# feinanshan/TDNet

Measured on AMD Instinct MI355X. Metric: frames/sec (td4-psp18, 1024x2048, full-resolution logits), higher is better.
Workload: dtype f32; 1 GPU; td4-psp18, 1024x2048 Cityscapes-shaped synthetic stream, 3-frame feature cache, 1 clip per GPU; parallelism=clip-parallel x1, RCCL weight broadcast only, target_fps_per_gpu=30

## Files before the change

include/tdnet.h:

```cpp
#ifndef TDNET_H
#define TDNET_H

#include <stddef.h>
#include <stdint.h>

#ifdef __cplusplus
extern "C" {
#endif

typedef struct tdnet tdnet_t;

typedef struct tdnet_cfg {
    int32_t model;
    int32_t backbone;
    int32_t nclass;
    int32_t height;
    int32_t width;
    int32_t device;
} tdnet_cfg;

#define TDNET_WINOGRAD_DEFAULT 3
#define TDNET_ATTENTION_DEFAULT 2
#define TDNET_FUSION_LN_STATS 2
#define TDNET_FUSION_LN_IN_HEAD 4
#define TDNET_FUSION_A_DIRECT 32
#define TDNET_FUSION_DMA_LOADERS 8192
#define TDNET_FUSION_DMA_NARROW 32768
#define TDNET_FUSION_STEM_ROWS 65536
#define TDNET_FUSION_CONV_GROUPS 131072
#define TDNET_FUSION_CLS_IN_HEAD 262144
#define TDNET_FUSION_SPLIT_NARROW 524288
#define TDNET_FUSION_LATE_CHAIN 1048576
#define TDNET_OVERLAP_CHAINS 1
#define TDNET_OVERLAP_LOWREG_TRANSFORMS 2
#define TDNET_OVERLAP_CHAINS_ANY_SIZE 4
#define TDNET_OVERLAP_GEMM_DMA 8
#define TDNET_OVERLAP_VW_SHIFT 4
#define TDNET_OVERLAP_VW_MASK 0x30
#define TDNET_FUSION_DEFAULT (TDNET_FUSION_LN_STATS | TDNET_FUSION_LN_IN_HEAD | TDNET_FUSION_A_DIRECT | TDNET_FUSION_DMA_LOADERS | TDNET_FUSION_DMA_NARROW | \
                              TDNET_FUSION_STEM_ROWS | TDNET_FUSION_CONV_GROUPS | TDNET_FUSION_CLS_IN_HEAD | TDNET_FUSION_SPLIT_NARROW | TDNET_FUSION_LATE_CHAIN)
#define TDNET_FUSION_MASK TDNET_FUSION_DEFAULT
#define TDNET_OVERLAP_DEFAULT (TDNET_OVERLAP_CHAINS | TDNET_OVERLAP_GEMM_DMA | (2 << TDNET_OVERLAP_VW_SHIFT))
#define TDNET_OVERLAP_MASK (TDNET_OVERLAP_CHAINS | TDNET_OVERLAP_LOWREG_TRANSFORMS | TDNET_OVERLAP_CHAINS_ANY_SIZE | TDNET_OVERLAP_GEMM_DMA | TDNET_OVERLAP_VW_MASK)
typedef struct tdnet_opts {
    int32_t winograd;
    int32_t precision;
    int32_t pipeline;
    int32_t gemm_persistent;
    int32_t reserved0;
    int32_t attention;
    int32_t fusion;
    int32_t overlap;
    int32_t reserved[8];
} tdnet_opts;
void tdnet_opts_default(tdnet_opts* o);

typedef struct tdnet_arch {
    int32_t dilated;
    int32_t multi_grid;
    int32_t reserved[6];
} tdnet_arch;
void tdnet_arch_default(tdnet_arch* a);

int  tdnet_create(const tdnet_cfg* cfg, tdnet_t** out);
int  tdnet_create_opts(const tdnet_cfg* cfg, const tdnet_opts* opts , tdnet_t** out);
int  tdnet_create_arch(const tdnet_cfg* cfg, const tdnet_arch* arch , const tdnet_opts* opts ,
                       tdnet_t** out);
int  tdnet_get_opts(const tdnet_t* h, tdnet_opts* out);
int  tdnet_get_arch(const tdnet_t* h, tdnet_arch* out);
int  tdnet_feature_dims(const tdnet_t* h, int* height, int* width);
void tdnet_destroy(tdnet_t* h);

int  tdnet_set_weight(tdnet_t* h, const char* name, const float* host, size_t count);
int  tdnet_finalize_weights(tdnet_t* h);
int  tdnet_create_shared(const tdnet_t* weights_of, const tdnet_opts* opts , tdnet_t** out);
int  tdnet_warmup(tdnet_t* h, void* stream);
int  tdnet_memory_bytes(const tdnet_t* h, size_t* weights_bytes, size_t* handle_bytes);

int  tdnet_forward(tdnet_t* h, const float* img_nchw_dev, int pos_id, float* logits_nchw_dev, void* stream);
int  tdnet_argmax(tdnet_t* h, const float* logits_nchw_dev, int32_t* labels_dev, void* stream);
int  tdnet_forward_labels(tdnet_t* h, const float* img_nchw_dev, int pos_id, int32_t* labels_dev, void* stream);
int  tdnet_set_input_u8(tdnet_t* h, int src_height, int src_width, const double* mean , const double* std );
int  tdnet_forward_u8(tdnet_t* h, const uint8_t* img_hwc_dev, int pos_id, float* logits_nchw_dev, void* stream);
int  tdnet_forward_u8_labels(tdnet_t* h, const uint8_t* img_hwc_dev, int pos_id, uint8_t* labels_dev , void* stream);
int  tdnet_argmax_u8(tdnet_t* h, const float* logits_nchw_dev, uint8_t* labels_dev, void* stream);
int  tdnet_set_output_rgb(tdnet_t* h, int out_height, int out_width, const uint8_t* palette_rgb , int n_colours );
int  tdnet_forward_rgb(tdnet_t* h, const float* img_nchw_dev, int pos_id, uint8_t* rgb_dev, void* stream);
int  tdnet_forward_u8_rgb(tdnet_t* h, const uint8_t* img_hwc_dev, int pos_id, uint8_t* rgb_dev, void* stream);
int  tdnet_labels_rgb(tdnet_t* h, const uint8_t* labels_u8_dev, uint8_t* rgb_dev, void* stream);
int  tdnet_set_score(tdnet_t* h, const uint8_t* gt_map );
int  tdnet_forward_score(tdnet_t* h, const float* img_nchw_dev, int pos_id, const uint8_t* gt_u8_dev, uint8_t* labels_u8_dev , void* stream);
int  tdnet_forward_u8_score(tdnet_t* h, const uint8_t* img_hwc_dev, int pos_id, const uint8_t* gt_u8_dev, uint8_t* labels_u8_dev , void* stream);
int  tdnet_labels_score(tdnet_t* h, const uint8_t* labels_u8_dev, const uint8_t* gt_u8_dev, void* stream);
// ... 34 lines not shown
```

tdnet_amd/_capi.py:

```python
import ctypes
import os

_HERE = os.path.dirname(os.path.abspath(__file__))
DEFAULT_LIB = os.path.join(_HERE, "lib", "libtdnet_hip.so")
TEST_LIB = os.path.join(_HERE, "lib", "libtdnet_hip_test.so")

c_float_p = ctypes.POINTER(ctypes.c_float)
c_void_p = ctypes.c_void_p


class TdnetCfg(ctypes.Structure):
    _fields_ = [("model", ctypes.c_int32), ("backbone", ctypes.c_int32), ("nclass", ctypes.c_int32),
                ("height", ctypes.c_int32), ("width", ctypes.c_int32), ("device", ctypes.c_int32)]


class TdnetOpts(ctypes.Structure):
    _fields_ = [("winograd", ctypes.c_int32), ("precision", ctypes.c_int32), ("pipeline", ctypes.c_int32),
                ("gemm_persistent", ctypes.c_int32), ("reserved0", ctypes.c_int32), ("attention", ctypes.c_int32),
                ("fusion", ctypes.c_int32), ("overlap", ctypes.c_int32), ("reserved", ctypes.c_int32 * 8)]

    def as_dict(self):
        return {k: getattr(self, k) for k, _ in self._fields_ if not k.startswith("reserved")}


# ... 43 lines not shown
    "tdnet_forward_u8_rgb": (ctypes.c_int, [c_void_p, c_void_p, ctypes.c_int, c_void_p, c_void_p]),
    "tdnet_labels_rgb": (ctypes.c_int, [c_void_p, c_void_p, c_void_p, c_void_p]),
    "tdnet_propagate_rgb": (ctypes.c_int, [c_void_p, c_void_p, c_void_p]),
    "tdnet_set_score": (ctypes.c_int, [c_void_p, c_void_p]),
    "tdnet_forward_score": (ctypes.c_int, [c_void_p, c_void_p, ctypes.c_int, c_void_p, c_void_p, c_void_p]),
    "tdnet_forward_u8_score": (ctypes.c_int, [c_void_p, c_void_p, ctypes.c_int, c_void_p, c_void_p, c_void_p]),
    "tdnet_propagate_score": (ctypes.c_int, [c_void_p, c_void_p, c_void_p, c_void_p]),
    "tdnet_labels_score": (ctypes.c_int, [c_void_p, c_void_p, c_void_p, c_void_p]),
    "tdnet_score_reset": (ctypes.c_int, [c_void_p, c_void_p]),
    "tdnet_score_export": (ctypes.c_int, [c_void_p, c_void_p, c_void_p]),
    "tdnet_score_read": (ctypes.c_long, [c_void_p, c_void_p, ctypes.c_size_t, c_void_p]),
    "tdnet_reset": (ctypes.c_int, [c_void_p]),
    "tdnet_fifo_len": (ctypes.c_int, [c_void_p]),
    "tdnet_encode": (ctypes.c_int, [c_void_p, c_void_p, ctypes.c_int, c_void_p]),
    "tdnet_propagate": (ctypes.c_int, [c_void_p, c_void_p, c_void_p]),
    "tdnet_propagate_labels": (ctypes.c_int, [c_void_p, c_void_p, c_void_p]),
    "tdnet_cache_dims": (ctypes.c_int, [c_void_p, ctypes.POINTER(ctypes.c_int), ctypes.POINTER(ctypes.c_int), ctypes.POINTER(ctypes.c_int)]),
    "tdnet_cache_export": (ctypes.c_int, [c_void_p, c_void_p, c_void_p, c_void_p, c_void_p]),
    "tdnet_cache_push": (ctypes.c_int, [c_void_p, c_void_p, c_void_p, c_void_p, c_void_p]),
    "tdnet_get_stage": (ctypes.c_long, [c_void_p, ctypes.c_char_p, c_void_p, ctypes.c_size_t]),
    "tdnet_flops_per_frame": (ctypes.c_double, [c_void_p]),
    "tdnet_set_profiling": (ctypes.c_int, [c_void_p, ctypes.c_int]),
    "tdnet_last_ms": (ctypes.c_double, [c_void_p, ctypes.c_int]),
    "tdnet_last_flops": (ctypes.c_double, [c_void_p, ctypes.c_int]),
    "tdnet_last_launches": (ctypes.c_double, [c_void_p, ctypes.c_int]),
    "tdnet_last_error": (ctypes.c_char_p, []),
    "tdnet_version": (ctypes.c_char_p, []),
}


TEST_SYMBOLS = {
    "tdnet_bench_mfma_peak": (ctypes.c_double, [ctypes.c_int, ctypes.c_int, c_void_p]),
    "tdnet_bench_conv": (ctypes.c_double, [ctypes.c_int] * 9 + [c_opts_p, c_void_p]),
    "tdnet_op_conv2d": (ctypes.c_int, [c_void_p, ctypes.c_int, ctypes.c_int, ctypes.c_int, c_void_p, c_void_p, ctypes.c_int,
                                       ctypes.c_int, ctypes.c_int, ctypes.c_int, c_void_p, ctypes.c_int, c_opts_p, ctypes.c_int,
                                       c_void_p, c_void_p]),
    "tdnet_op_conv2d_f16io": (ctypes.c_int, [c_void_p, ctypes.c_int, ctypes.c_int, ctypes.c_int, c_void_p, c_void_p, ctypes.c_int,
                                             ctypes.c_int, ctypes.c_int, ctypes.c_int, c_void_p, ctypes.c_int, ctypes.c_int,
                                             c_void_p, c_void_p]),
    "tdnet_op_stem": (ctypes.c_int, [c_void_p, ctypes.c_int, ctypes.c_int, c_void_p, c_void_p, c_opts_p, c_void_p, c_void_p]),
    "tdnet_op_attention": (ctypes.c_int, [c_void_p, c_void_p, c_void_p, c_void_p, c_void_p, ctypes.c_int, ctypes.c_int,
                                          ctypes.c_int, ctypes.c_int, c_void_p, c_void_p, c_void_p, c_void_p, c_void_p]),
    "tdnet_op_layernorm_hw": (ctypes.c_int, [c_void_p, ctypes.c_int, ctypes.c_int, c_void_p, c_void_p, c_void_p, c_void_p]),
    "tdnet_op_ppm": (ctypes.c_int, [c_void_p, ctypes.c_int, ctypes.c_int, c_void_p, c_void_p, ctypes.c_int, ctypes.c_int,
                                    c_void_p, c_void_p]),
    "tdnet_op_upsample": (ctypes.c_int, [c_void_p, ctypes.c_int, ctypes.c_int, ctypes.c_int, ctypes.c_int, ctypes.c_int,
                                         c_void_p, c_void_p]),
    "tdnet_op_stem_image": (ctypes.c_long, [c_void_p, c_void_p, ctypes.c_int, ctypes.c_int, ctypes.c_int, ctypes.c_int, ctypes.POINTER(ctypes.c_double),
                                            ctypes.POINTER(ctypes.c_double), ctypes.c_int, c_void_p, ctypes.c_size_t, c_void_p]),
    "tdnet_op_upsample_argmax": (ctypes.c_int, [c_void_p, ctypes.c_int, ctypes.c_int, ctypes.c_int, ctypes.c_int, ctypes.c_int, c_void_p, c_void_p, c_void_p]),
    "tdnet_op_upsample_argmax_rgb": (ctypes.c_int, [c_void_p] + [ctypes.c_int] * 7 + [c_void_p, ctypes.c_int, c_void_p, c_void_p, c_void_p]),
    "tdnet_op_upsample_argmax_score": (ctypes.c_int, [c_void_p] + [ctypes.c_int] * 5 + [c_void_p] * 6),
    "tdnet_op_nearest_index": (ctypes.c_int, [ctypes.c_int, ctypes.c_int, c_void_p]),
    "tdnet_op_classifier": (ctypes.c_int, [c_void_p, ctypes.c_int, ctypes.c_int, c_void_p, c_void_p, ctypes.c_int, c_void_p, c_void_p]),
    "tdnet_op_head_cls": (ctypes.c_int, [c_void_p, ctypes.c_int, ctypes.c_int, ctypes.c_int, c_void_p, c_void_p, ctypes.c_int, ctypes.c_int,
                                         c_void_p, c_void_p, ctypes.c_int, c_opts_p, ctypes.c_int, c_void_p, c_void_p]),
}


class Lib:

    def __init__(self, path=DEFAULT_LIB, test_symbols=False):
        if not os.path.exists(path):
            raise TdnetError("HIP library not found: %s -- build it with `python -c 'import __graft_entry__ as g; g.build()'` "
                             "(hipcc --offload-arch=gfx950); there is no CPU fallback" % path)
        self.path = path
        if path in (DEFAULT_LIB, TEST_LIB):
            import torch
        self.dll = ctypes.CDLL(path)
        for name, (res, args) in list(SYMBOLS.items()) + (list(TEST_SYMBOLS.items()) if test_symbols else []):
            fn = getattr(self.dll, name)
            fn.restype = res
            fn.argtypes = args
            setattr(self, name, fn)

    def opts(self, **kw):
        o = TdnetOpts()
        self.tdnet_opts_default(ctypes.byref(o))
        for k, v in kw.items():
            if k not in dict(TdnetOpts._fields_) or k.startswith("reserved"):
                raise TypeError("unknown tdnet_opts field %r" % k)
            if v is not None:
                setattr(o, k, int(v))
        return o

    def arch(self, dilated=True, multi_grid=True):
        a = TdnetArch()
        self.tdnet_arch_default(ctypes.byref(a))
        a.dilated, a.multi_grid = int(bool(dilated)), int(bool(multi_grid))
        return a

    def check(self, rc):
        if rc is not None and rc < 0:
            raise TdnetError(self.tdnet_last_error().decode())
        return rc


_default = None
_test = None


def lib():
    global _default
    if _default is None:
        _default = Lib(DEFAULT_LIB)
    return _default
# ... 8 lines not shown
```

tdnet_amd/csrc/td_handle.h:

```cpp
#pragma once
#include "../../include/tdnet.h"
#include "td_device.h"
#include "td_conv.h"
#include "td_conv_h.h"
#include "td_conv_hd.h"
#include "td_conv_ad.h"
#include "td_wino.h"
#include "td_gemm.h"
#include "td_gemm_dma.h"
#include "td_gemm_b3.h"
#include "td_conv_ad_b3.h"
#include "td_attn.h"
#include "td_attn_h.h"
#include "td_attn_b3.h"
#include "td_misc.h"
#include "td_ingest.h"
#include "td_score.h"

#include <cmath>
#include <cstdarg>
#include <cstdio>
#include <algorithm>
#include <atomic>
#include <cstring>
#include <cstdlib>
#include <map>
#include <string>
#include <vector>

static thread_local char g_err[1024] = "";
static int td_fail(const char* fmt, ...) {
    va_list ap;
    va_start(ap, fmt);
    vsnprintf(g_err, sizeof(g_err), fmt, ap);
    va_end(ap);
    return -1;
}
#define TD_HIP(expr)                                                                            \
    do {                                                                                        \
        hipError_t e_ = (expr);                                                                 \
        if (e_ != hipSuccess) return td_fail("%s failed: %s (%s:%d)", #expr, hipGetErrorString(e_), __FILE__, __LINE__); \
    } while (0)

#define TD_TRY(expr) do { if ((expr) != 0) return -1; } while (0)

struct DevGuard {
    int prev = -1;
    bool switched = false, ok = true;
    explicit DevGuard(int dev) {
        if (hipGetDevice(&prev) != hipSuccess) { ok = false; return; }
        if (prev != dev) { ok = hipSetDevice(dev) == hipSuccess; switched = ok; }
    }
    ~DevGuard() { if (switched) (void)hipSetDevice(prev); }
};
#define TD_ON_DEVICE(n, ...)                                                                      \
    DevGuard dev_guard_((n)->cfg.device);                                                         \
    if (!dev_guard_.ok) { td_fail("cannot select HIP device %d", (n)->cfg.device); return __VA_ARGS__; }

struct BlockSpec { std::string name; int cin, cout, stride, dil1, dil2; bool ds; bool bott; int planes; };

// ... 1 lines not shown
    const int nb18[4] = {2, 2, 2, 2}, nb34[4] = {3, 4, 6, 3};
    const int nb101[4] = {3, 4, 23, 3};
    const int* nb = backbone == 18 ? nb18 : backbone == 101 ? nb101 : nb34;
    const bool bott = backbone == 50 || backbone == 101;
    const int exp = bott ? 4 : 1;
    const int planes[4] = {64, 128, 256, 512};
    const int strides[4] = {1, 2, dilated ? 1 : 2, dilated ? 1 : 2}, dils[4] = {1, 1, dilated ? 2 : 1, dilated ? 4 : 1};
    std::vector<BlockSpec> out;
    int inpl = bott ? 128 : 64;
    for (int li = 0; li < 4; ++li) {
        for (int b = 0; b < nb[li]; ++b) {
            const bool first = b == 0, mg = li == 3 && dilated && multi_grid;
            int d1;
            if (mg) d1 = b == 0 ? 4 : b == 1 ? 8 : 16;
            else if (first) d1 = (dils[li] == 1 || dils[li] == 2) ? 1 : 2;
            else d1 = dils[li];
            BlockSpec s;
            char nm[32];
            snprintf(nm, sizeof(nm), "layer%d.%d", li + 1, b);
            s.name = nm;
            s.cin = first ? inpl : planes[li] * exp;
            s.cout = planes[li] * exp;
            s.bott = bott;
            s.planes = planes[li];
            s.stride = first ? strides[li] : 1;
            s.dil1 = d1;
            s.dil2 = dils[li];
            s.ds = first && (strides[li] != 1 || inpl != planes[li] * exp);
            out.push_back(s);
        }
        inpl = planes[li] * exp;
    }
    return out;
}
static int key_size(int n) { return (n - 1) / 4 + 1; }
static int out_size(int n, int KS, int stride, int dil, int pad) { return (n + 2 * pad - dil * (KS - 1) - 1) / stride + 1; }
static int feature_size(int n, const std::vector<BlockSpec>& blocks) {
    n = (n - 1) / 2 + 1;
    n = (n - 1) / 2 + 1;
    for (const BlockSpec& s : blocks) n = out_size(n, 3, s.stride, s.dil1, s.dil1);
    return n;
}

enum ConvRoute {
    CR_IGEMM,
    CR_ADIRECT,
    CR_ADIRECT_ROWS,
    CR_ADIRECT_B3,
    CR_ADIRECT_ROWS_B3,
    CR_GEMM1X1,
    CR_STEM_H,
    CR_CONV_H,
    CR_CONV_DMA,
    CR_WINO
};
enum GemmKernel {
    GK_CONV,
    GK_PERSISTENT,
    GK_DMA,
    GK_B3
};
struct ConvLayer {
    int Cin = 0, Cout = 0, KS = 1, stride = 1, dil = 1, pad = 0, act = 0;
    bool stem = false;
    ConvRoute route = CR_IGEMM;
    GemmKernel gemm = GK_CONV;
    bool in16 = false, out16 = false;
    int rh = 0;
    bool rowimg_off = false;
    int pers = 1;
    int chunks = 1;
    int vw = 0;
    int wino = 0;
    float* d_zero = nullptr;
    ConvTile tile = CT_128x128;
    int CoutPad = 0, nsteps = 0;
    float* d_wp = nullptr;
    float* d_bias = nullptr;
    bool h16() const { return route == CR_STEM_H || route == CR_CONV_H || route == CR_CONV_DMA; }
    bool stem_rows() const { return route == CR_ADIRECT_ROWS || route == CR_ADIRECT_ROWS_B3; }
    double flops_per_pixel() const { return 2.0 * Cout * (stem ? 3.0 * KS * KS : (double)Cin * KS * KS); }
};

static_assert(TDNET_FUSION_DEFAULT == 2072614 && TDNET_FUSION_MASK == 2072614 && TDNET_OVERLAP_DEFAULT == 41 && TDNET_OVERLAP_MASK == 0x3f,
              "the named option bits of include/tdnet.h must add up to the documented values");
static tdnet_opts opts_or_default(const tdnet_opts* o) {
    tdnet_opts d;
    tdnet_opts_default(&d);
    if (!o) return d;
    d = *o;
    d.winograd = d.winograd <= 0 ? 0 : (d.winograd == 2 || d.winograd >= 4) ? 4 : 3;
    d.precision = d.precision < 0 ? 0 : d.precision > 3 ? 1 : d.precision;
    d.pipeline = d.pipeline ? 1 : 0;
    d.gemm_persistent = d.gemm_persistent < 0 ? 0 : d.gemm_persistent;
    d.attention = d.attention < 0 ? 0 : d.attention > 2 ? 2 : d.attention;
    d.fusion &= TDNET_FUSION_MASK;
    d.overlap = d.overlap < 0 ? 0 : d.overlap & TDNET_OVERLAP_MASK;
    if ((d.overlap & TDNET_OVERLAP_VW_MASK) == TDNET_OVERLAP_VW_MASK) d.overlap &= ~TDNET_OVERLAP_VW_MASK;
    d.reserved0 = 0;
    for (int& r : d.reserved) r = 0;
    return d;
}

struct BlockLayers { ConvLayer c1, c2, c3, ds; bool has_ds = false, bott = false; };
struct AtnLayer { ConvLayer fc; float* d_bias = nullptr; };
struct PathLayers {
    ConvLayer stem, stem2, stem3;
    std::vector<BlockLayers> blocks;
    float* d_ppm_w = nullptr; float* d_ppm_b = nullptr;
    ConvLayer enc_v, enc_q0, enc_q1, enc_k0, enc_k1;
    std::vector<AtnLayer> atn;
    float* d_ln_g = nullptr; float* d_ln_b = nullptr;
    ConvLayer head3;
    float* d_cls_w = nullptr; float* d_cls_b = nullptr;
    int pid = 0;
};
struct CacheSlot { float* q = nullptr; float* k = nullptr; float* v = nullptr; };
struct U8Input {
    bool set = false;
    int Hs = 0, Ws = 0, H = 0, W = 0, Wt = 0;
    double mean[3] = {0, 0, 0}, std[3] = {1, 1, 1};
    bool resize = false;
    int span = 0, threads = 256;
    float* lut = nullptr;
    int* xt = nullptr;
    int* yt = nullptr;
    size_t bytes = 0;
};
struct RgbOutput {
    bool set = false;
    int H = 0, W = 0, oh = 0, ow = 0, n_colours = 0;
    unsigned char palette[768] = {0};
    int* ys = nullptr;
    int* xs = nullptr;
    unsigned* lut = nullptr;
    size_t bytes = 0;
};
// ... 249 lines not shown
```

tdnet_amd/csrc/td_launch.h:

```cpp
#pragma once
#include "td_weights.h"

#ifdef TDNET_TIMING_PROBES
static int probe_skip() {
    static const int m = [] {
        const char* e = getenv("TDNET_PROBE_SKIP");
        const int v = e ? atoi(e) : 0;
        if (v) fprintf(stderr, "tdnet: TDNET_PROBE_SKIP=%d -- pieces of the frame are NOT computed, every result of this process is garbage (timing probe build)\n", v);
        return v;
    }();
    return m;
}
#else
static constexpr int probe_skip() { return 0; }
#endif
static void prof_begin(tdnet* n, int family, int dominant, double flops, hipStream_t s) {
    if (!n || !n->prof) return;
    if (n->nrec == n->recs.size()) {
        ProfRec r;
        hipEventCreate(&r.e0); hipEventCreate(&r.e1);
        n->recs.push_back(r);
    }
    ProfRec& r = n->recs[n->nrec];
    r.family = family; r.dominant = dominant; r.flops = flops;
// ... 74 lines not shown
            if (L.Cout == 128) TD_LAUNCH((k_wino4_out_cls<2>), dim3(grid), dim3(256), wino_out_cls_lds(128, cls->NC), s, wa, *cls);
            else TD_LAUNCH((k_wino4_out_cls<1>), dim3(grid), dim3(256), wino_out_cls_lds(64, cls->NC), s, wa, *cls);
        } else
        if (L.vw == 1) launch_wino4_c<1>(out_side, wa, s);
        else if (L.vw == 2 && C % 2 == 0) launch_wino4_c<2>(out_side, wa, s);
        else if (L.vw == 4 && C % 4 == 0) launch_wino4_c<4>(out_side, wa, s);
        else if (L.vw) launch_wino4_c<1>(out_side, wa, s);
        else if (out_side && wino_act_general(wa.act)) TD_LAUNCH((k_wino4_out<true>), dim3(td_grid_for(T * (L.Cout / 4), 256, 256 * 16)), dim3(256), 0, s, wa);
        else if (out_side) TD_LAUNCH((k_wino4_out<false>), dim3(td_grid_for(T * (L.Cout / 4), 256, 256 * 16)), dim3(256), 0, s, wa);
        else TD_LAUNCH(k_wino4_in, dim3(td_grid_for(T * (L.Cin / 4), 256, 256 * 16)), dim3(256), 0, s, wa);
        prof_end(n, s);
    };
    transform(false);
    prof_begin(n, 0, 2, 2.0 * nb * Tc * (double)L.Cin * L.Cout, s);
    if (!(n && (probe_skip() & 8))) launch_gemm(L, gemm_args(L, V, (int)Tc, nb, L.d_zero, nullptr, Mb, 0), chunked ? 320 : 0, s);
    prof_end(n, s);
    transform(true);
    if (own) { TD_HIP(hipStreamSynchronize(s)); hipFree(V); hipFree(Mb); }
    return 0;
}

static void launch_conv_dma_forms(const ConvLayer& L, const ConvArgs& a, hipStream_t s) {
    int rh = L.rh;
    bool done = false;
    const bool is192 = rh == CD_192_P || rh == CD_192_N;
    if (rh == CD_128_N || rh == CD_192_N) {
        done = !L.rowimg_off && conv_launch_dma3n(a, rh, L.KS, L.out16, s);
        if (!done) rh = is192 ? CD_192_P : CD_128_P;
    }
    if (!done && (rh == CD_128_P || rh == CD_192_P)) {
        done = !L.rowimg_off && conv_launch_dma3p(a, rh, L.KS, L.out16, s);
        if (!done) rh = is192 ? CD_192 : CD_128_8W;
    }
    if (!done && (L.rowimg_off || !conv_launch_dma3(a, rh, L.KS, L.out16, s))) conv_launch_dma(a, rh, L.KS, L.out16, s);
}

static int run_conv(tdnet* n, const ConvLayer& L, const float* in, int H, int W, const float* resid, float* out, hipStream_t s,
                    int* Ho_out = nullptr, int* Wo_out = nullptr, const LnFuse* lnf = nullptr, const ClsArgs* cls = nullptr) {
    if (lnf && !L.wino) return td_fail("internal: LayerNorm fusion needs a Winograd input transform");
    if (cls && (!L.wino || L.chunks > 1 || resid || wino_act_general(L.act))) return td_fail("internal: the classifier rides in a whole Winograd conv's output transform");
    const int Ho = out_size(H, L.KS, L.stride, L.dil, L.pad), Wo = out_size(W, L.KS, L.stride, L.dil, L.pad);
    if (L.wino) {
        if (Ho_out) *Ho_out = H;
        if (Wo_out) *Wo_out = W;
        if (L.chunks > 1 && (!n || !n->ws_ready)) {
            for (int c = 0; c < L.chunks; ++c) {
                WinoChunk ck; ck.ny = L.chunks; ck.cy = c;
                TD_TRY(run_wino(n, L, in, H, W, resid, out, s, lnf, ck, nullptr, nullptr));
            }
            return 0;
        }
        return run_wino(n, L, in, H, W, resid, out, s, lnf, WinoChunk(), nullptr, nullptr, cls);
    }
    const ConvArgs a = conv_args(L, in, H, W, resid, out);
    prof_begin(n, 0, (((L.tile == CT_128x128 || L.tile == CT_128x128_DEEP || L.rh) && L.KS == 3 && !L.stem) ? 1 : 0) | ((L.h16() && L.in16 && L.KS == 3 && !L.stem) ? 4 : 0), L.flops_per_pixel() * a.M, s);
    switch (L.route) {
    case CR_STEM_H: conv_launch_stem_h(a, L.out16, s); break;
    case CR_CONV_DMA: launch_conv_dma_forms(L, a, s); break;
    case CR_CONV_H: conv_launch_h(a, L.tile, L.KS, L.in16, L.out16, s); break;
    case CR_ADIRECT_B3: conv_launch_adirect_b3(a, L.KS, 0, s); break;
    case CR_GEMM1X1: launch_gemm(L, gemm_args(L, in, a.M, 1, L.d_bias, resid, out, L.act), 0, s); break;
    case CR_ADIRECT_ROWS:
    case CR_ADIRECT_ROWS_B3: {
        ConvArgs r = a;
        r.H = stem_rows_hp(H); r.W = stem_rows_wp(W); r.Cin = 3; r.pad = 0;
        if (L.route == CR_ADIRECT_ROWS_B3) conv_launch_adirect_b3(r, L.KS, 2, s);
        else conv_launch_adirect(r, L.KS, 2, s);
        break;
    }
    case CR_ADIRECT: conv_launch_adirect(a, L.KS, L.stem ? 1 : 0, s); break;
    case CR_IGEMM: conv_launch(a, L.tile, L.KS, L.stem, s); break;
    case CR_WINO: break;
    }
    prof_end(n, s);
    if (Ho_out) *Ho_out = Ho;
    if (Wo_out) *Wo_out = Wo;
    return 0;
}

struct ConvCall { const ConvLayer* L; const float* in; int H, W; float* out; };
static int run_conv_group(tdnet* n, const ConvCall* c, int ng, hipStream_t s, int* Ho_out = nullptr, int* Wo_out = nullptr) {
    bool same = n && (n->opts.fusion & TDNET_FUSION_CONV_GROUPS) && ng >= 2 && ng <= 3;
    for (int g = 0; same && g < ng; ++g) {
        const ConvLayer& L = *c[g].L;
        const ConvLayer& L0 = *c[0].L;
        same = L.route == CR_CONV_H && L.in16 == L.out16 && L.in16 == L0.in16 && (g == 0 ? (L.KS == 1 || L.KS == 3) : L.KS == 1) &&
               conv_tile_dims(L.tile).BM == conv_tile_dims(L0.tile).BM && conv_tile_dims(L.tile).BN == conv_tile_dims(L0.tile).BN;
    }
    if (!same) {
        for (int g = 0; g < ng; ++g) TD_TRY(run_conv(n, *c[g].L, c[g].in, c[g].H, c[g].W, nullptr, c[g].out, s, g == 0 ? Ho_out : nullptr, g == 0 ? Wo_out : nullptr));
        return 0;
    }
    ConvArgs a[3];
    double flops = 0.0;
    for (int g = 0; g < ng; ++g) {
        const ConvLayer& L = *c[g].L;
        a[g] = conv_args(L, c[g].in, c[g].H, c[g].W, nullptr, c[g].out);
        flops += L.flops_per_pixel() * a[g].M;
        if (g == 0 && Ho_out) *Ho_out = out_size(c[0].H, L.KS, L.stride, L.dil, L.pad);
        if (g == 0 && Wo_out) *Wo_out = a[0].Wo;
    }
    const bool dom = c[0].L->in16 && c[0].L->KS == 3;
    prof_begin(n, 0, dom ? 4 : 0, dom ? c[0].L->flops_per_pixel() * a[0].M : flops, s);
    conv_launch_h_group(a, ng, c[0].L->tile, c[0].L->KS, c[0].L->in16, c[0].L->out16, s);
    prof_end(n, s);
    return 0;
}

static int run_attention(tdnet* n, const float* q, const float* k, const float* vp, const float* bias, const float* resid,
                         int Lq, int Lk, int DV, float* out, hipStream_t s, int online = 0, float* ln_part = nullptr,
                         _Float16* vt16 = nullptr, bool slices = false, bool vt_ready = false, int b3 = 0) {
    if (n && n->vt16 && (n->opts.precision == 1 || b3)) vt16 = n->vt16;
    AttnArgs a;
    a.q = q; a.k = k; a.vp = vp; a.bias = bias; a.resid = resid; a.out = out; a.Lq = Lq; a.Lk = Lk;
    a.scale_log2e = 1.4426950408889634f / 8.0f;
    a.ln_part = ln_part; a.ln_nstr = 0;
    if (n && (probe_skip() & 4) && Lq > Lk) return 0;
    prof_begin(n, 1, false, 2.0 * Lq * (double)Lk * (64 + DV), s);
    const int rc = (vt16 && b3) ? attn_launch_b3(a, DV, reinterpret_cast<unsigned short*>(vt16), s, vt_ready, b3 - 1)
                 : vt16 ? attn_launch_h(a, DV, vt16, s, vt_ready) : attn_launch(a, DV, online, s, slices);
    prof_end(n, s);
    if (rc) return td_fail("attention: unsupported d_v=%d (128 or a multiple of 512)", DV);
    return 0;
}

// ... 125 lines not shown
```

tdnet_amd/csrc/td_weights.h:

```cpp
#pragma once
#include "td_handle.h"

constexpr int RH_FRAME = -1;
constexpr int RH_BY_SIZE = -2;

static int plan_dma_form(const ConvLayer& c, long M, const tdnet_opts& o) {
    const bool narrow = (o.fusion & TDNET_FUSION_DMA_NARROW) != 0, same3 = c.KS == 3 && c.stride == 1 && c.pad == c.dil;
    if (!conv_dma_supports(c.Cin, c.Cout, c.KS, c.tile)) return CD_NONE;
    if (c.Cout == 64 && c.CoutPad == 128 && same3 && narrow) return CD_128_N;
    if (c.Cout < 128) return CD_NONE;
    const int rh = conv_dma_pick_rh(M, c.Cout, c.CoutPad % 256 == 0);
    if (narrow && same3 && M <= 16384 && c.Cout <= 256) return c.Cout <= 128 ? CD_128_N : CD_192_N;
    if (o.fusion & TDNET_FUSION_DMA_LOADERS) return rh == CD_128 ? CD_128_P : rh == CD_192 ? CD_192_P : rh;
    return rh;
}

static int plan_conv(ConvLayer& L, int Cout, int Cin, int KS, int stride, int dil, int act, bool stem, long M, const tdnet_opts& o,
                     int forced_tile = -1, int chunks = 1, bool in16 = false, bool out16 = false, int rh = RH_FRAME, bool rowimg_off = false) {
    L = ConvLayer();
    L.Cin = stem ? 4 : Cin; L.Cout = Cout; L.KS = KS; L.stride = stride; L.dil = dil; L.act = act; L.stem = stem;
    L.pad = stem ? KS / 2 : dil * (KS / 2);
    L.pers = o.gemm_persistent;
    L.rowimg_off = rowimg_off;
    if (!stem && Cin % 32 != 0) return td_fail("conv: Cin=%d is not a multiple of 32", Cin);
    const bool deep = o.pipeline != 0, forced = forced_tile >= 0;
    const bool pers_gemm = o.gemm_persistent && gemm_supports(Cin);
    const bool split = o.precision >= 2;
    const bool split_narrow = split && (o.fusion & TDNET_FUSION_A_DIRECT) && (o.fusion & TDNET_FUSION_SPLIT_NARROW);
    if (o.winograd && o.precision != 1 && !stem && KS == 3 && stride == 1 && Cin % 32 == 0 && Cout % 4 == 0 && (o.winograd == 4 || (Cin >= 128 && Cout >= 128))) {
        L.route = CR_WINO;
        L.wino = 4;
        L.chunks = (chunks > 1 && dil % chunks == 0 && pers_gemm) ? chunks : 1;
        L.vw = (L.chunks > 1 || (o.overlap & TDNET_OVERLAP_LOWREG_TRANSFORMS)) ? (1 << ((o.overlap & TDNET_OVERLAP_VW_MASK) >> TDNET_OVERLAP_VW_SHIFT)) : 0;
        const int nb = (L.wino + 2) * (L.wino + 2);
        const long rows = wino_tiles_estimate(M, dil, L.wino) / L.chunks;
        L.tile = forced ? (ConvTile)forced_tile : pers_gemm ? gemm_pick_tile(rows, nb, Cout, deep)
                                                            : conv_pick_tile((int)std::min<long>(nb * M / (L.wino * L.wino), 1 << 30), Cout, deep);
        L.nsteps = conv_nsteps(Cin, 1, 0);
        const bool b3 = split && pers_gemm && gemm_b3_supports(Cin, Cout) && (forced || o.precision == 3 || gemm_b3_pick(rows, nb, Cout));
        L.gemm = !pers_gemm ? GK_CONV : b3 ? GK_B3 : ((o.overlap & TDNET_OVERLAP_GEMM_DMA) && gemm_dma_supports(Cin, Cout, L.tile)) ? GK_DMA : GK_PERSISTENT;
        L.CoutPad = b3 ? gemm_b3_npad(Cout) : conv_cout_pad(Cout, L.tile);
        return 0;
    }
    const bool h16 = o.precision == 1 && !stem && Cin % 64 == 0;
    const bool stem16 = o.precision == 1 && stem && KS == 7 && stride == 2 && Cout <= 64;
    const bool is1x1 = !h16 && !stem && KS == 1 && stride == 1 && pers_gemm;
    const bool narrow1x1 = is1x1 && !forced && split_narrow && Cout <= 128 && M >= 8192 && gemm_b3_supports(Cin, Cout) && !gemm_b3_pick(M, 1, Cout, Cin) &&
                           conv_adirect_b3_supports(CT_128x64, Cin, KS, stem);
    const bool gemm1x1 = is1x1 && !narrow1x1;
    L.tile = forced ? (ConvTile)forced_tile : gemm1x1 ? gemm_pick_tile(M, 1, Cout, deep) : conv_pick_tile((int)M, Cout, deep);
    if (!forced && split_narrow && !h16 && !stem && !gemm1x1 && Cout <= 128 && conv_adirect_b3_supports(CT_128x64, Cin, KS, stem)) L.tile = CT_128x64;
    if (h16 && !forced && (o.fusion & TDNET_FUSION_DMA_NARROW) && KS == 3 && stride == 1 && Cout == 64) L.tile = CT_128x128_DEEP;
    L.CoutPad = conv_cout_pad(Cout, L.tile);
    L.nsteps = conv_nsteps(Cin, KS, stem ? 1 : 0);
    if (stem16 && conv_stem_h_supports(L.tile)) {
        L.route = CR_STEM_H;
        L.nsteps = conv_nsteps_stem_h();
    } else if (h16) {
        L.route = CR_CONV_H;
        L.nsteps = conv_nsteps_h(Cin, KS);
    } else if (gemm1x1) {
        const bool b3 = split && gemm_b3_supports(Cin, Cout) && (forced || o.precision == 3 || gemm_b3_pick(M, 1, Cout, Cin));
        L.route = CR_GEMM1X1;
        L.gemm = b3 ? GK_B3 : GK_PERSISTENT;
        if (b3) { L.CoutPad = gemm_b3_npad(Cout); L.nsteps = Cin / 16; }
    } else if (split_narrow && conv_adirect_b3_supports(L.tile, Cin, KS, stem)) {
        L.route = CR_ADIRECT_B3;
    } else if ((o.fusion & TDNET_FUSION_A_DIRECT) && conv_adirect_supports(L.tile, 1)) {
        const bool rows = stem && KS == 7 && stride == 2 && (o.fusion & TDNET_FUSION_STEM_ROWS);
        L.route = !rows ? CR_ADIRECT : split_narrow ? CR_ADIRECT_ROWS_B3 : CR_ADIRECT_ROWS;
        if (rows) L.nsteps = conv_nsteps(Cin, KS, 2);
    }
    if (L.h16()) { L.in16 = in16; L.out16 = out16; }
    if (L.route == CR_CONV_H && L.in16) {
        L.rh = rh == RH_FRAME ? plan_dma_form(L, M, o)
             : rh == RH_BY_SIZE ? (Cout >= 128 && conv_dma_supports(Cin, Cout, KS, L.tile) ? conv_dma_pick_rh(M, Cout, L.CoutPad % 256 == 0) : CD_NONE) : rh;
        if (L.rh) L.route = CR_CONV_DMA;
    }
    return 0;
}

template <typename T, typename Pack>
static int upload_packed(float** d, size_t count, Pack pack) {
    std::vector<T> packed(count);
    pack(packed.data());
    TD_TRY(dev_alloc((T**)d, count));
    TD_HIP(hipMemcpy(*d, packed.data(), count * sizeof(T), hipMemcpyHostToDevice));
    return 0;
}
static int upload_conv(ConvLayer& L, const std::vector<float>& w, const std::vector<float>& b) {
    typedef unsigned short bf16;
    const int Cout = L.Cout, Cin = L.Cin, KS = L.KS, stem_kind = L.stem_rows() ? 2 : L.stem ? 1 : 0;
    const size_t tile_image = (size_t)L.nsteps * 8 * L.CoutPad * 4;
    if (L.route == CR_WINO) {
        const int nb = (L.wino + 2) * (L.wino + 2);
        std::vector<std::vector<float>> U;
        wino_transform_weights(w.data(), Cout, Cin, L.wino, U);
        const size_t per = L.gemm == GK_B3 ? gemm_b3_packed_bytes(Cin, Cout) / 2 : tile_image;
        if (L.gemm == GK_B3) TD_TRY(upload_packed<bf16>(&L.d_wp, nb * per, [&](bf16* p) { for (int bi = 0; bi < nb; ++bi) gemm_b3_pack(U[bi].data(), Cout, Cin, p + bi * per); }));
        else TD_TRY(upload_packed<float>(&L.d_wp, nb * per, [&](float* p) { for (int bi = 0; bi < nb; ++bi) conv_pack_weights(U[bi].data(), Cout, Cin, 1, 0, L.tile, p + bi * per); }));
    } else if (L.route == CR_STEM_H)
        TD_TRY(upload_packed<_Float16>(&L.d_wp, 2 * tile_image, [&](_Float16* p) { conv_pack_weights_stem_h(w.data(), Cout, L.tile, p); }));
    else if (L.h16())
        TD_TRY(upload_packed<_Float16>(&L.d_wp, 2 * tile_image, [&](_Float16* p) { conv_pack_weights_h(w.data(), Cout, Cin, KS, L.tile, p); }));
    else if (L.route == CR_GEMM1X1 && L.gemm == GK_B3)
        TD_TRY(upload_packed<bf16>(&L.d_wp, gemm_b3_packed_bytes(Cin, Cout) / 2, [&](bf16* p) { gemm_b3_pack(w.data(), Cout, Cin, p); }));
    else if (L.route == CR_ADIRECT_B3 || L.route == CR_ADIRECT_ROWS_B3)
        TD_TRY(upload_packed<bf16>(&L.d_wp, conv_adb3_packed_bytes(Cout, Cin, KS, stem_kind) / 2, [&](bf16* p) { conv_pack_weights_adb3(w.data(), Cout, Cin, KS, p, stem_kind); }));
    else
        TD_TRY(upload_packed<float>(&L.d_wp, tile_image, [&](float* p) { conv_pack_weights(w.data(), Cout, Cin, KS, stem_kind, L.tile, p); }));
    TD_TRY(upload(&L.d_bias, b.empty() ? std::vector<float>(Cout, 0.f) : b));
    if (L.wino) TD_TRY(upload(&L.d_zero, std::vector<float>(Cout, 0.f)));
    return 0;
}
static void free_conv_layer(ConvLayer& L) {
    if (L.d_wp) hipFree(L.d_wp);
    if (L.d_bias) hipFree(L.d_bias);
    if (L.d_zero) hipFree(L.d_zero);
    L.d_wp = L.d_bias = L.d_zero = nullptr;
}
static void add_bn(std::map<std::string, size_t>& e, const std::string& pre, int c) {
    e[pre + ".weight"] = c; e[pre + ".bias"] = c; e[pre + ".running_mean"] = c; e[pre + ".running_var"] = c;
    e[pre + ".num_batches_tracked"] = 1;
}
static std::vector<std::string> atn_module_names(int model) {
    if (model == 4) return {"atn1_2", "atn1_3", "atn1_4", "atn2_1", "atn2_3", "atn2_4", "atn3_1", "atn3_2", "atn3_4", "atn4_1", "atn4_2", "atn4_3"};
    return {"atn1", "atn2"};
}
static std::vector<std::string> atn_order(int model, int p) {
    if (model == 2) return {p == 0 ? "atn1" : "atn2"};
    static const char* t[4][3] = {{"atn1_2", "atn1_3", "atn1_4"}, {"atn2_3", "atn2_4", "atn2_1"},
                                  {"atn3_4", "atn3_1", "atn3_2"}, {"atn4_1", "atn4_2", "atn4_3"}};
    return {t[p][0], t[p][1], t[p][2]};
}
static void build_expected(tdnet* n) {
    auto& e = n->expected;
    char b[160];
    for (int p = 1; p <= n->P; ++p) {
        snprintf(b, sizeof(b), "pretrained%d", p);
        std::string pre = n->cfg.model == 1 ? std::string("pretrained") : std::string(b);
        if (n->deep) {
            e[pre + ".conv1.0.weight"] = 64 * 3 * 9; add_bn(e, pre + ".conv1.1", 64);
            e[pre + ".conv1.3.weight"] = 64 * 64 * 9; add_bn(e, pre + ".conv1.4", 64);
            e[pre + ".conv1.6.weight"] = 128 * 64 * 9; add_bn(e, pre + ".bn1", 128);
        } else {
            e[pre + ".conv1.weight"] = 64 * 3 * 49;
            add_bn(e, pre + ".bn1", 64);
        }
        for (auto& s : n->bspec) {
            std::string bp = pre + "." + s.name;
            if (s.bott) {
                e[bp + ".conv1.weight"] = (size_t)s.planes * s.cin; add_bn(e, bp + ".bn1", s.planes);
                e[bp + ".conv2.weight"] = (size_t)s.planes * s.planes * 9; add_bn(e, bp + ".bn2", s.planes);
// ... 373 lines not shown
```

Before: 284.8 frames/s.

## Add fused single-kernel Winograd F(4,3) path for 64-channel 3x3 convs

Adds a new conv route that runs the whole Winograd F(4x4,3x3) convolution for 64-in/64-out channel layers in one kernel. The kernel does the input transform, the per-position MFMA GEMM and the output transform with bias, residual and activation, staging intermediates in LDS. This removes the separate transform and GEMM launches and the global round trips for transformed tiles on these narrow layers. The route is enabled by default for fp32 precision when the layer is large enough. It adds a new specialised kernel with heavy register use (9 accumulators of 16 floats) and a different reduction order than the existing path.

```diff
diff --git a/include/tdnet.h b/include/tdnet.h
--- a/include/tdnet.h
+++ b/include/tdnet.h
@@ -31,6 +31,7 @@
 #define TDNET_FUSION_CLS_IN_HEAD 262144
 #define TDNET_FUSION_SPLIT_NARROW 524288
 #define TDNET_FUSION_LATE_CHAIN 1048576
+#define TDNET_FUSION_WINO_FUSED_64 2097152
 #define TDNET_OVERLAP_CHAINS 1
 #define TDNET_OVERLAP_LOWREG_TRANSFORMS 2
 #define TDNET_OVERLAP_CHAINS_ANY_SIZE 4
@@ -38,7 +39,8 @@
 #define TDNET_OVERLAP_VW_SHIFT 4
 #define TDNET_OVERLAP_VW_MASK 0x30
 #define TDNET_FUSION_DEFAULT (TDNET_FUSION_LN_STATS | TDNET_FUSION_LN_IN_HEAD | TDNET_FUSION_A_DIRECT | TDNET_FUSION_DMA_LOADERS | TDNET_FUSION_DMA_NARROW | \
-                              TDNET_FUSION_STEM_ROWS | TDNET_FUSION_CONV_GROUPS | TDNET_FUSION_CLS_IN_HEAD | TDNET_FUSION_SPLIT_NARROW | TDNET_FUSION_LATE_CHAIN)
+                              TDNET_FUSION_STEM_ROWS | TDNET_FUSION_CONV_GROUPS | TDNET_FUSION_CLS_IN_HEAD | TDNET_FUSION_SPLIT_NARROW | TDNET_FUSION_LATE_CHAIN | \
+                              TDNET_FUSION_WINO_FUSED_64)
 #define TDNET_FUSION_MASK TDNET_FUSION_DEFAULT
 #define TDNET_OVERLAP_DEFAULT (TDNET_OVERLAP_CHAINS | TDNET_OVERLAP_GEMM_DMA | (2 << TDNET_OVERLAP_VW_SHIFT))
 #define TDNET_OVERLAP_MASK (TDNET_OVERLAP_CHAINS | TDNET_OVERLAP_LOWREG_TRANSFORMS | TDNET_OVERLAP_CHAINS_ANY_SIZE | TDNET_OVERLAP_GEMM_DMA | TDNET_OVERLAP_VW_MASK)
diff --git a/tdnet_amd/_capi.py b/tdnet_amd/_capi.py
--- a/tdnet_amd/_capi.py
+++ b/tdnet_amd/_capi.py
@@ -119,6 +119,7 @@
     "tdnet_op_upsample_argmax_rgb": (ctypes.c_int, [c_void_p] + [ctypes.c_int] * 7 + [c_void_p, ctypes.c_int, c_void_p, c_void_p, c_void_p]),
     "tdnet_op_upsample_argmax_score": (ctypes.c_int, [c_void_p] + [ctypes.c_int] * 5 + [c_void_p] * 6),
     "tdnet_op_nearest_index": (ctypes.c_int, [ctypes.c_int, ctypes.c_int, c_void_p]),
+    "tdnet_op_launch_count": (ctypes.c_long, []),
     "tdnet_op_classifier": (ctypes.c_int, [c_void_p, ctypes.c_int, ctypes.c_int, c_void_p, c_void_p, ctypes.c_int, c_void_p, c_void_p]),
     "tdnet_op_head_cls": (ctypes.c_int, [c_void_p, ctypes.c_int, ctypes.c_int, ctypes.c_int, c_void_p, c_void_p, ctypes.c_int, ctypes.c_int,
                                          c_void_p, c_void_p, ctypes.c_int, c_opts_p, ctypes.c_int, c_void_p, c_void_p]),
diff --git a/tdnet_amd/csrc/td_handle.h b/tdnet_amd/csrc/td_handle.h
--- a/tdnet_amd/csrc/td_handle.h
+++ b/tdnet_amd/csrc/td_handle.h
@@ -6,6 +6,7 @@
 #include "td_conv_hd.h"
 #include "td_conv_ad.h"
 #include "td_wino.h"
+#include "td_wino_fused.h"
 #include "td_gemm.h"
 #include "td_gemm_dma.h"
 #include "td_gemm_b3.h"
@@ -113,7 +114,8 @@
     CR_STEM_H,
     CR_CONV_H,
     CR_CONV_DMA,
-    CR_WINO
+    CR_WINO,
+    CR_WINO_FUSED
 };
 enum GemmKernel {
     GK_CONV,
@@ -143,7 +145,7 @@
     double flops_per_pixel() const { return 2.0 * Cout * (stem ? 3.0 * KS * KS : (double)Cin * KS * KS); }
 };
 
-static_assert(TDNET_FUSION_DEFAULT == 2072614 && TDNET_FUSION_MASK == 2072614 && TDNET_OVERLAP_DEFAULT == 41 && TDNET_OVERLAP_MASK == 0x3f,
+static_assert(TDNET_FUSION_DEFAULT == 4169766 && TDNET_FUSION_MASK == 4169766 && TDNET_OVERLAP_DEFAULT == 41 && TDNET_OVERLAP_MASK == 0x3f,
               "the named option bits of include/tdnet.h must add up to the documented values");
 static tdnet_opts opts_or_default(const tdnet_opts* o) {
     tdnet_opts d;
diff --git a/tdnet_amd/csrc/td_launch.h b/tdnet_amd/csrc/td_launch.h
--- a/tdnet_amd/csrc/td_launch.h
+++ b/tdnet_amd/csrc/td_launch.h
@@ -150,6 +150,18 @@
         }
         return run_wino(n, L, in, H, W, resid, out, s, lnf, WinoChunk(), nullptr, nullptr, cls);
     }
+    if (L.route == CR_WINO_FUSED) {
+        if (!wino_fused_fits((long)H * W)) return td_fail("internal: this conv is too large for the fused Winograd kernel");
+        WinoFusedArgs fa;
+        fa.in = in; fa.wf = L.d_wp; fa.bias = L.d_bias; fa.resid = resid; fa.out = out;
+        fa.H = H; fa.W = W; fa.TY = wino_tiles_1d(H, 1, 4); fa.TX = wino_tiles_1d(W, 1, 4); fa.T = fa.TY * fa.TX; fa.act = L.act;
+        prof_begin(n, 0, 0, 2.0 * 36 * fa.T * (double)L.Cin * L.Cout, s);
+        wino_fused_launch(fa, s);
+        prof_end(n, s);
+        if (Ho_out) *Ho_out = H;
+        if (Wo_out) *Wo_out = W;
+        return 0;
+    }
     const ConvArgs a = conv_args(L, in, H, W, resid, out);
     prof_begin(n, 0, (((L.tile == CT_128x128 || L.tile == CT_128x128_DEEP || L.rh) && L.KS == 3 && !L.stem) ? 1 : 0) | ((L.h16() && L.in16 && L.KS == 3 && !L.stem) ? 4 : 0), L.flops_per_pixel() * a.M, s);
     switch (L.route) {
@@ -168,7 +180,7 @@
     }
     case CR_ADIRECT: conv_launch_adirect(a, L.KS, L.stem ? 1 : 0, s); break;
     case CR_IGEMM: conv_launch(a, L.tile, L.KS, L.stem, s); break;
-    case CR_WINO: break;
+    case CR_WINO: case CR_WINO_FUSED: break;
     }
     prof_end(n, s);
     if (Ho_out) *Ho_out = Ho;
diff --git a/tdnet_amd/csrc/td_weights.h b/tdnet_amd/csrc/td_weights.h
--- a/tdnet_amd/csrc/td_weights.h
+++ b/tdnet_amd/csrc/td_weights.h
@@ -14,6 +14,8 @@
     if (o.fusion & TDNET_FUSION_DMA_LOADERS) return rh == CD_128 ? CD_128_P : rh == CD_192 ? CD_192_P : rh;
     return rh;
 }
+
+constexpr long TD_WINO_FUSED_MIN_PIXELS = 74000;
 
 static int plan_conv(ConvLayer& L, int Cout, int Cin, int KS, int stride, int dil, int act, bool stem, long M, const tdnet_opts& o,
                      int forced_tile = -1, int chunks = 1, bool in16 = false, bool out16 = false, int rh = RH_FRAME, bool rowimg_off = false) {
@@ -27,6 +29,12 @@
     const bool pers_gemm = o.gemm_persistent && gemm_supports(Cin);
     const bool split = o.precision >= 2;
     const bool split_narrow = split && (o.fusion & TDNET_FUSION_A_DIRECT) && (o.fusion & TDNET_FUSION_SPLIT_NARROW);
+    if (o.precision == 0 && o.winograd && (o.fusion & TDNET_FUSION_WINO_FUSED_64) && !stem && !forced && wino_fused_supports(Cin, Cout, KS, stride, dil) &&
+        wino_fused_fits(M) && !wino_act_general(act) && (o.winograd == 4 || M >= TD_WINO_FUSED_MIN_PIXELS)) {
+        L.route = CR_WINO_FUSED;
+        L.CoutPad = Cout;
+        return 0;
+    }
     if (o.winograd && o.precision != 1 && !stem && KS == 3 && stride == 1 && Cin % 32 == 0 && Cout % 4 == 0 && (o.winograd == 4 || (Cin >= 128 && Cout >= 128))) {
         L.route = CR_WINO;
         L.wino = 4;
@@ -99,6 +107,10 @@
         const size_t per = L.gemm == GK_B3 ? gemm_b3_packed_bytes(Cin, Cout) / 2 : tile_image;
         if (L.gemm == GK_B3) TD_TRY(upload_packed<bf16>(&L.d_wp, nb * per, [&](bf16* p) { for (int bi = 0; bi < nb; ++bi) gemm_b3_pack(U[bi].data(), Cout, Cin, p + bi * per); }));
         else TD_TRY(upload_packed<float>(&L.d_wp, nb * per, [&](float* p) { for (int bi = 0; bi < nb; ++bi) conv_pack_weights(U[bi].data(), Cout, Cin, 1, 0, L.tile, p + bi * per); }));
+    } else if (L.route == CR_WINO_FUSED) {
+        std::vector<std::vector<float>> U;
+        wino_transform_weights(w.data(), Cout, Cin, 4, U);
+        TD_TRY(upload_packed<float>(&L.d_wp, (size_t)36 * Cout * Cin, [&](float* p) { wino_fused_pack(U, p); }));
     } else if (L.route == CR_STEM_H)
         TD_TRY(upload_packed<_Float16>(&L.d_wp, 2 * tile_image, [&](_Float16* p) { conv_pack_weights_stem_h(w.data(), Cout, L.tile, p); }));
     else if (L.h16())
diff --git a/tdnet_amd/csrc/td_wino_fused.h b/tdnet_amd/csrc/td_wino_fused.h
--- /dev/null
+++ b/tdnet_amd/csrc/td_wino_fused.h
@@ -0,0 +1,168 @@
+#pragma once
+#include "td_wino.h"
+
+struct WinoFusedArgs {
+    const float* in;
+    const float* wf;
+    const float* bias;
+    const float* resid;
+    float* out;
+    int H, W, TY, TX, T, act;
+};
+constexpr int TD_WF_C = 64;
+constexpr int TD_WF_KQ = 32 * 4 + 4;
+constexpr int TD_WF_POS = 4 * TD_WF_KQ;
+constexpr int TD_WF_LDS = 36 * TD_WF_POS * 4;
+constexpr unsigned TD_WF_WPOS = 16u * 64u * 16u;
+
+TD_DEV void td_wf_patch(const WinoFusedArgs& p, int tile, unsigned chan_bytes, unsigned (&offy)[6], unsigned (&offx)[6]) {
+    const int ty = tile / p.TX, tx = tile - ty * p.TX;
+    const bool live = tile < p.T;
+#pragma unroll
+    for (int r = 0; r < 6; ++r) {
+        const int y = 4 * ty - 1 + r, x = 4 * tx - 1 + r;
+        offy[r] = (live && (unsigned)y < (unsigned)p.H) ? (unsigned)y * (unsigned)p.W * (TD_WF_C * 4u) : TD_BUF_OOB;
+        offx[r] = (unsigned)x < (unsigned)p.W ? (unsigned)x * (TD_WF_C * 4u) + chan_bytes : TD_BUF_OOB;
+    }
+}
+
+TD_KERNEL void TD_LAUNCH_BOUNDS(256, 2) k_wino4_fused64(WinoFusedArgs p) {
+    TD_DYN_LDS(smem);
+    float* lds = reinterpret_cast<float*>(smem);
+    const int tid = threadIdx.x, lane = tid & 63, wave = td_wave();
+    const int half = lane >> 5, l31 = lane & 31;
+    const int grp = blockIdx.x >> 4, rem = blockIdx.x & 15;
+    const int blk = grp * 8 + (rem & 7), nh = rem >> 3;
+    if (blk * 32 >= p.T) return;
+    const int t0 = blk * 32;
+    const unsigned pix_bytes = (unsigned)p.H * (unsigned)p.W * (TD_WF_C * 4u);
+    const TdBuf in_buf = td_make_buf(p.in, pix_bytes);
+    const TdBuf w_buf = td_make_buf(p.wf, 36u * TD_WF_WPOS);
+
+    f32x16 acc[9];
+#pragma unroll
+    for (int i = 0; i < 9; ++i)
+#pragma unroll
+        for (int r = 0; r < 16; ++r) acc[i][r] = 0.f;
+
+    const int ch = lane & 15, tl = lane >> 4;
+    const float* As = lds + half * TD_WF_KQ + l31 * 4;
+    const unsigned b_lane = (unsigned)((half * 64 + nh * 32 + l31) * 16);
+
+    for (int c = 0; c < 4; ++c) {
+#pragma unroll
+        for (int pass = 0; pass < 2; ++pass) {
+            const int tb = 16 * pass + 4 * tl + wave;
+            unsigned offy[6], offx[6];
+            td_wf_patch(p, t0 + tb, (unsigned)(16 * c + ch) * 4u, offy, offx);
+            float dd[6][6];
+#pragma unroll
+            for (int cc = 0; cc < 6; ++cc)
+#pragma unroll
+                for (int r = 0; r < 6; ++r) dd[cc][r] = td_buf_ld1(in_buf, __builtin_elementwise_add_sat(offy[r], offx[cc]), 0u);
+            float tm[6][6];
+#pragma unroll
+            for (int cc = 0; cc < 6; ++cc) {
+                float col[6];
+                td_wino4_bt_t(dd[cc], col);
+#pragma unroll
+                for (int r = 0; r < 6; ++r) tm[r][cc] = col[r];
+            }
+            float* vs = lds + (ch >> 2) * TD_WF_KQ + tb * 4 + (ch & 3);
+#pragma unroll
+            for (int r = 0; r < 6; ++r) {
+                float v[6];
+                td_wino4_bt_t(tm[r], v);
+#pragma unroll
+                for (int cc = 0; cc < 6; ++cc) vs[(r * 6 + cc) * TD_WF_POS] = v[cc];
+            }
+        }
+        __syncthreads();
+#pragma unroll
+        for (int i = 0; i < 9; ++i) {
+            const int pos = 9 * wave + i;
+#pragma unroll
+            for (int g = 0; g < 2; ++g) {
+                const f32x4 a = td_ld4(As + pos * TD_WF_POS + 2 * g * TD_WF_KQ);
+                const f32x4 b = td_buf_ld4(w_buf, b_lane, (unsigned)pos * TD_WF_WPOS + (unsigned)(4 * c + 2 * g) * 1024u);
+#pragma unroll
+                for (int s = 0; s < 4; ++s) acc[i] = td_mfma32(a[s], b[s], acc[i]);
+            }
+        }
+        __syncthreads();
+    }
+
+    const TdBuf res_buf = td_make_buf(p.resid, p.resid ? pix_bytes : 0u);
+    const TdBuf out_buf = td_make_buf(p.out, pix_bytes);
+    const TdBuf bias_buf = td_make_buf(p.bias, TD_WF_C * 4u);
+#pragma unroll
+    for (int q = 0; q < 2; ++q) {
+        if (q) __syncthreads();
+        if ((l31 >> 4) == q) {
+            float* ms = lds + 9 * wave * TD_WF_POS + 4 * half * 16 + (l31 & 15);
+#pragma unroll
+            for (int i = 0; i < 9; ++i)
+#pragma unroll
+                for (int r = 0; r < 16; ++r) ms[i * TD_WF_POS + ((r & 3) + 8 * (r >> 2)) * 16] = acc[i][r];
+        }
+        __syncthreads();
+        const int co = nh * 32 + q * 16 + ch;
+        const float b = td_buf_ld1(bias_buf, (unsigned)co * 4u, 0u);
+#pragma unroll
+        for (int pass = 0; pass < 2; ++pass) {
+            const int tb = 8 * wave + 4 * pass + tl;
+            const int tile = t0 + tb, ty = tile / p.TX, tx = tile - ty * p.TX;
+            unsigned offy[4], offx[4];
+#pragma unroll
+            for (int r = 0; r < 4; ++r) {
+                const int y = 4 * ty + r, x = 4 * tx + r;
+                offy[r] = (tile < p.T && y < p.H) ? (unsigned)y * (unsigned)p.W * (TD_WF_C * 4u) : TD_BUF_OOB;
+                offx[r] = x < p.W ? ((unsigned)x * TD_WF_C + (unsigned)co) * 4u : TD_BUF_OOB;
+            }
+            float o[16];
+#pragma unroll
+            for (int r = 0; r < 4; ++r)
+#pragma unroll
+                for (int cc = 0; cc < 4; ++cc) o[r * 4 + cc] = td_buf_ld1(res_buf, __builtin_elementwise_add_sat(offy[r], offx[cc]), 0u);
+            const float* mr = lds + tb * 16 + ch;
+            float mm[6][6];
+#pragma unroll
+            for (int cc = 0; cc < 6; ++cc)
+#pragma unroll
+                for (int r = 0; r < 6; ++r) mm[cc][r] = mr[(r * 6 + cc) * TD_WF_POS];
+            float sm[4][6];
+#pragma unroll
+            for (int cc = 0; cc < 6; ++cc) {
+                float col[4];
+                td_wino4_at_t(mm[cc], col);
+#pragma unroll
+                for (int r = 0; r < 4; ++r) sm[r][cc] = col[r];
+            }
+#pragma unroll
+            for (int r = 0; r < 4; ++r) {
+                float o4[4];
+                td_wino4_at_t(sm[r], o4);
+#pragma unroll
+                for (int cc = 0; cc < 4; ++cc) o[r * 4 + cc] = (o4[cc] + b) + o[r * 4 + cc];
+            }
+            td_wino_activate<false>(o, p.act);
+#pragma unroll
+            for (int r = 0; r < 4; ++r)
+#pragma unroll
+                for (int cc = 0; cc < 4; ++cc) td_buf_st1(out_buf, __builtin_elementwise_add_sat(offy[r], offx[cc]), 0u, o[r * 4 + cc]);
+        }
+    }
+}
+
+static inline bool wino_fused_supports(int Cin, int Cout, int KS, int stride, int dil) { return Cin == TD_WF_C && Cout == TD_WF_C && KS == 3 && stride == 1 && dil == 1; }
+static inline bool wino_fused_fits(long M) { return M * TD_WF_C * 4 < (1l << 31); }
+static inline void wino_fused_pack(const std::vector<std::vector<float>>& U, float* dst) {
+    for (int pos = 0; pos < 36; ++pos)
+        for (int kq = 0; kq < 16; ++kq)
+            for (int co = 0; co < TD_WF_C; ++co)
+                for (int e = 0; e < 4; ++e) dst[(((size_t)pos * 16 + kq) * TD_WF_C + co) * 4 + e] = U[pos][(size_t)co * TD_WF_C + kq * 4 + e];
+}
+static inline void wino_fused_launch(const WinoFusedArgs& a, hipStream_t s) {
+    const int nblk = (a.T + 31) / 32;
+    TD_LAUNCH(k_wino4_fused64, dim3((unsigned)((nblk + 7) / 8 * 16)), dim3(256), TD_WF_LDS, s, a);
+}
```

New measurement: 290.8 frames/s, median of 6. +2.1%, better.
